# ChicyChen/LOCO-Edit

Hardware: AMD Instinct MI355X
Metric: edit-directions/sec (top-5 PMP-Jacobian SVD @256^2) + vT cos-sim vs ref (higher is better)
Workload: dtype bf16x3 (split-bf16 MFMA operands, fp32 accumulate + fp32 storage); 1 GPU; CelebA-HQ DDPM 256x256 top-5 local basis (l_eye-sized mask, L=2400), t=0.6T, 12 power iterations, one GPU; multi_gpu_form=single, probes_total=5, probes_per_gpu=5, kept=5, n_iter=12, mask_L=2400, weights=synthetic seed 0, streams=2

## Files before the change

loco-edit_amd/csrc/engine.hip:

```cpp
#include <hip/hip_runtime.h>

#include <algorithm>
#include <array>
#include <cmath>
#include <cstdio>
#include <cstdlib>
#include <cstring>
#include <map>
#include <memory>
#include <thread>
#include <atomic>
#include <string>
#include <vector>

#include "../../include/loco_hip.h"
#ifdef LOCO_DIAG
#include "../../include/loco_hip_diag.h"
#endif
#include "kernels.h"
#include "program.h"
#ifdef LOCO_DIAG
#include "conv_plan_text.h"
#endif

// ... 464 lines not shown
        switch (op.kind) {
            case OP_CONV_IN: case OP_CONV: case OP_DOWN: case OP_UP: case OP_OUT: convf(ow.conv, to.H, to.W); break;
            case OP_RES:
                convf(ow.c1, to.H, to.W); convf(ow.c2, to.H, to.W);
                if (op.has_nin) convf(ow.nin, to.H, to.W);
                break;
            case OP_XFMR: {
                for (const ConvP* p : {&ow.pj_in, &ow.qkvc, &ow.to_out1, &ow.xqc, &ow.to_out2, &ow.ff1, &ow.ff2, &ow.pj_out}) convf(*p, to.H, to.W);
                double T = (double)to.H * to.W;
                fl += 2.0 * 2.0 * T * T * to.C + 2.0 * 2.0 * T * c->cfg.context_len * to.C;
                break;
            }
            case OP_ATTN: {
                convf(ow.qkvc, to.H, to.W); convf(ow.proj, to.H, to.W);
                double T = (double)to.H * to.W;
                fl += 2.0 * 2.0 * T * T * to.C;
                if (op.has_x) {
                    convf(ow.xqc, to.H, to.W); convf(ow.xproj, to.H, to.W);
                    fl += 2.0 * 2.0 * T * c->cfg.context_len * to.C;
                }
                break;
            }
        }
    }
    W.flops = fl;
    for (auto& kv : c->params) { std::vector<float>().swap(kv.second.data); }
    return bind_weights(c);
}

struct Pass {
    loco_ctx* c;
    hipStream_t st;
    int B;
    float* arena;
    float* stats;
    float* T(int id) const { return arena + c->tens[id].off; }
    long bs() const { return c->prog->per_sample; }
};

static void drop_graphs(loco_ctx* c) {
    for (auto& kv : c->fwd_graphs) {
        if (kv.second.exec) (void)hipGraphExecDestroy(kv.second.exec);
        if (kv.second.graph) (void)hipGraphDestroy(kv.second.graph);
    }
    c->fwd_graphs.clear();
}
inline unsigned char* gemm_ws_get(loco_ctx* c, size_t need, hipStream_t st) {
    const int l = c->lane;
    if (c->gemm_ws_bytes[l] >= need) return c->gemm_ws[l];
    hipStreamCaptureStatus cs = hipStreamCaptureStatusNone;
    if (hipStreamIsCapturing(st, &cs) != hipSuccess || cs != hipStreamCaptureStatusNone) return nullptr;
    if (c->gemm_ws[l]) {
        (void)hipDeviceSynchronize();
        drop_graphs(c);
        (void)hipFree(c->gemm_ws[l]);
        c->bytes -= c->gemm_ws_bytes[l];
        c->gemm_ws[l] = nullptr; c->gemm_ws_bytes[l] = 0;
    }
    void* p = nullptr;
    if (hipMalloc(&p, need) != hipSuccess) { (void)hipGetLastError(); return nullptr; }
    c->gemm_ws[l] = static_cast<unsigned char*>(p); c->gemm_ws_bytes[l] = need; c->bytes += need;
    return c->gemm_ws[l];
}
inline void attn_note(loco_ctx* c, const char* kernel, const GemmArgs* g = nullptr) {
#ifdef LOCO_DIAG
    if (!c->attn_log) return;
    char line[192];
    if (g) snprintf(line, sizeof(line), "kernel=%s M=%d N=%d K=%d batch=%d heads=%d kcat=%d\n", kernel, g->M, g->N, g->K, g->batch,
                    g->batch2 > 0 ? g->batch2 : 1, g->A2 ? 1 : 0);
    else snprintf(line, sizeof(line), "kernel=%s\n", kernel);
    *c->attn_log += line;
#else
    (void)c; (void)kernel; (void)g;
#endif
}
inline bool attn_gemm_rec(const loco_ctx* c, const GemmArgs& g) { return c->prec >= 1 && c->gemm_lowp && gemm_rec_eligible(g); }
inline void attn_gemm_f32(loco_ctx* c, const GemmArgs& g, hipStream_t st) { attn_note(c, "gemm_f32", &g); launch_gemm(g, st); }
inline void attn_gemm(loco_ctx* c, const GemmArgs& g, hipStream_t st) {
    if (attn_gemm_rec(c, g)) {
        if (unsigned char* ws = gemm_ws_get(c, gemm_rec_ws_bytes(g), st)) { attn_note(c, "gemm_rec", &g); launch_gemm_rec(g, ws, st); return; }
    }
    if (c->prec >= 1 && c->gemm_lowp && gemm_prefers_bf16x3(g)) { attn_note(c, "gemm_bf16x3", &g); launch_gemm_bf16x3(g, st); }
    else attn_gemm_f32(c, g, st);
}
inline void attn_softmax_rows(loco_ctx* c, float* S, long rows, int T, hipStream_t st, int B, long bs) {
    attn_note(c, "softmax_rows"); launch_softmax_rows(S, rows, T, st, B, bs);
}
inline void attn_softmax_jac(loco_ctx* c, float* dS, const float* P, long rows, int T, float scale, hipStream_t st, int B, long bs) {
    attn_note(c, "softmax_jac"); launch_softmax_jac(dS, P, rows, T, rows, scale, st, B, bs);
}

void conv_defaults(ConvArgs& a) {
    std::memset(&a, 0, sizeof(a));
    a.stride = 1; a.pad = 1; a.nsplit = 1; a.mode = CM_NONE; a.res_scale = 1.f;
}

struct NS { float *sc, *sh, *mr, *tst, *tc; };
NS nstats(const loco_ctx* c, float* base, const NormP& n) {
    NS s;
    s.sc = base + n.soff; s.sh = s.sc + n.C; s.mr = s.sh + n.C; s.tst = s.mr + 2 * c->cfg.gn_groups;
    s.tc = s.tst + 2 * c->cfg.gn_groups;
    return s;
}

struct StatReq {
    int kind = ST_NONE;
    NormP* n = nullptr;
    float* stats = nullptr;
    const float* prim = nullptr;
    const float* ss_scale = nullptr; const float* ss_shift = nullptr;
    float* keep = nullptr; size_t keep_floats = 0; int* keep_ntile = nullptr;
};

void stats_standalone(loco_ctx* c, const StatReq& rq, const float* x, long xbs, int B, int HW, int s0, hipStream_t st) {
    const NormP& n = *rq.n;
    const long SB = c->prog->stats_per_sample;
    const int G = c->cfg.gn_groups;
    if (rq.kind == ST_FWD) {
        NS s = nstats(c, rq.stats + (long)s0 * SB, n);
        launch_gn_stats(x, xbs, B, n.C, HW, G, eps_of(c, n), n.gamma, n.beta, s.mr, s.sc, s.sh, SB, c->red, st, rq.ss_scale,
                        rq.ss_shift);
    } else {
        NS sp = nstats(c, c->statsP, n);
        NS stt = nstats(c, rq.stats + (long)s0 * SB, n);
        launch_gn_tstats(x, xbs, rq.prim, 0, B, n.C, HW, G, sp.sc, sp.sh, sp.mr, 0, 0, rq.kind == ST_TAN ? 0 : 1, stt.tst,
                         stt.tc, SB, c->red, st, c->cfg.act);
    }
}

bool run_conv(loco_ctx* c, const ConvArgs& a0, int taps, hipStream_t st, const StatReq* rq = nullptr,
              const ConvArgs* second = nullptr) {
    const size_t span = (size_t)c->cfg.max_batch * c->prog->per_sample;
    auto padded = [&](const float* p) { return (p >= c->arenaP && p < c->arenaP + span) || (p >= c->arenaT && p < c->arenaT + span); };
    ConvArgs a = a0, sc;
    a.act = c->cfg.act;
    if (a.mode == CM_GN_SILU && c->cfg.act == ACT_GELU) a.mode = CM_GN_GELU;
    a.in_padded = padded(a.in);
    if (second) { sc = *second; sc.in_padded = padded(sc.in); }
    ConvEnv e;
    e.prec = c->prec; e.chip_share = c->chip_share; e.lanes = c->lanes_active; e.lane_s0 = c->lane_s0;
    e.partial = c->partial; e.partial_floats = c->partial_floats; e.stpart = c->stpart; e.stpart_floats = c->stpart_floats;
    e.fuse_stats = c->fuse_stats; e.fuse_lin = c->fuse_lin; e.deep1 = c->deep1; e.max_batch = c->cfg.max_batch;
    StatAsk q;
    if (rq) {
        q.kind = rq->kind; q.norm = rq->n != nullptr; q.prim = rq->prim; q.keep = rq->keep; q.keep_floats = rq->keep_floats;
        if (rq->n && rq->n->sx_off >= 0 && c->sxcache) q.sx = c->sxcache + rq->n->sx_off;
    }
    const ConvPlan p = plan_conv(e, a, taps, rq ? &q : nullptr, second ? &sc : nullptr);
    if (p.sc_first) run_conv(c, *second, 1, st);
#ifdef LOCO_DIAG
    if (c->plan_log) conv_plan_text(p, taps, c->prec, *c->plan_log);
#endif
    if (rq && rq->kind != ST_NONE && rq->n) rq->n->ready = true;
    if (rq && rq->keep_ntile) *rq->keep_ntile = p.keep_ntile;
    const int HWo = a.Hout * a.Wout, Gn = c->cfg.gn_groups;
    const long SBs = c->prog->stats_per_sample;
    auto timed = [&](const char* name, double flops, const ConvArgs& y, auto&& launch) {
        loco_ctx::ProfRec r;
        if (c->prof_on) {
            r.name = name; r.flops = flops;
            r.cin = y.Cin; r.cout = y.Cout; r.h = y.Hout; r.b = y.B; r.ns = y.nsplit; r.mode = y.mode; r.taps = taps;
            r.e0 = c->next_event(); r.e1 = c->next_event();
            (void)hipEventRecord(r.e0, st);
        }
        launch();
        if (c->prof_on) { (void)hipEventRecord(r.e1, st); c->prof.push_back(r); }
// ... 223 lines not shown
                     float beta, const float* V2 = nullptr, long vb2 = 0, const float* S2 = nullptr, long sb2 = 0) {
    const int n = text ? s.Lt : s.T, col0 = text ? 0 : s.Lt;
    GemmArgs g; std::memset(&g, 0, sizeof(g));
    g.A = V; g.sam = n; g.sak = 1; g.sab = vb; g.sah = text ? s.KS : s.HS;
    g.Bm = S + col0; g.sbk = 1; g.sbn = s.Tk; g.sbb = sb; g.sbh = s.SS;
    g.C = O; g.scm = s.T; g.scn = 1; g.scb = ob; g.sch = oh;
    g.M = s.CH; g.N = s.T; g.K = n; g.batch = s.B; g.batch2 = s.NH; g.alpha = 1.f; g.beta = beta;
    g.A2 = V2; g.sab2 = vb2; g.Bm2 = S2 ? S2 + col0 : nullptr; g.sbb2 = sb2;
    return g;
}
GemmArgs attn_keys(const Attn& s, const float* X, long xb, long xh, const float* S, long sb, float* G, long gb) {
    GemmArgs g; std::memset(&g, 0, sizeof(g));
    g.A = X; g.sam = s.T; g.sak = 1; g.sab = xb; g.sah = xh;
    g.Bm = S + s.Lt; g.sbk = s.Tk; g.sbn = 1; g.sbb = sb; g.sbh = s.SS;
    g.C = G; g.scm = s.T; g.scn = 1; g.scb = gb; g.sch = s.HS;
    g.M = s.CH; g.N = s.T; g.K = s.T; g.batch = s.B; g.batch2 = s.NH; g.alpha = 1.f; g.beta = 0.f;
    return g;
}
AttnFlashArgs attn_flash_args(const Attn& s) {
    AttnFlashArgs fa; std::memset(&fa, 0, sizeof(fa));
    fa.ws = s.ws; fa.ws_bytes = s.ws_bytes;
    fa.T = s.T; fa.NH = s.NH; fa.B = s.B; fa.CH = s.CH; fa.scale = s.scale;
    fa.q = s.q; fa.k = s.k; fa.v = s.v; fa.hs = s.HS;
    fa.P = s.P; fa.o = s.o;
    if (s.Lt) { fa.Lt = s.Lt; fa.kt = s.kt; fa.vt = s.vt; }
    return fa;
}
inline void attn_note_flash(loco_ctx* c, const AttnFlashArgs& fa, bool tan) {
#ifdef LOCO_DIAG
    if (!c->attn_log) return;
    const bool dma = attn_flash_dma_route(fa.ws, fa.ws_bytes, attn_flash_ws_bytes(fa), attn_flash_dma_enabled());
    if (dma) attn_note(c, "attn_split");
    if (tan) attn_note(c, dma ? "flash_dma_tan" : "flash_tan");
    else { attn_note(c, dma ? "flash_dma_cotq" : "flash_cotq"); attn_note(c, dma ? "flash_dma_cotk" : "flash_cotk"); }
#else
    (void)c; (void)fa; (void)tan;
#endif
}
void attn_forward(const Attn& s) {
    loco_ctx* c = s.c;
    float *q = s.tq, *k = s.tk, *v = s.tv, *S = s.tS, *o = s.to;
    if (s.Lt) attn_gemm_f32(c, attn_scores(s, TEXT, q, s.bq, s.HS, s.kt, 0, S, s.bS, s.scale, 0.f, true), s.st);
    attn_gemm(c, attn_scores(s, IMAGE, q, s.bq, s.HS, k, s.bq, S, s.bS, s.scale, 0.f), s.st);
    attn_softmax_rows(c, S, (long)s.NH * s.T, s.Tk, s.st, s.B, s.bS);
    attn_gemm(c, attn_values(s, IMAGE, v, s.bq, S, s.bS, o, s.bo, s.OS, 0.f), s.st);
    if (s.Lt) attn_gemm_f32(c, attn_values(s, TEXT, s.vt, 0, S, s.bS, o, s.bo, s.OS, 1.f), s.st);
}
void attn_tangent(const Attn& s) {
    loco_ctx* c = s.c;
    const float *q = s.q, *k = s.k, *v = s.v, *SP = s.P;
    float *dq = s.tq, *dk = s.tk, *dv = s.tv, *ST = s.tS, *oT = s.to;
    if (s.flash()) {
        AttnFlashArgs fa = attn_flash_args(s);
        fa.dq = dq; fa.dk = dk; fa.dv = dv; fa.bs_d = s.bq; fa.out = oT; fa.bs_out = s.bo;
        attn_note_flash(c, fa, true);
        launch_attn_flash_tangent(fa, s.st);
        return;
    }
    const GemmArgs dS2 = attn_scores(s, IMAGE, dq, s.bq, s.HS, k, 0, ST, s.bS, 1.f, 0.f, false, q, 0, dk, s.bq);
    const bool kcat = s.pair && (s.T <= 256 || attn_gemm_rec(c, dS2));
    if (s.Lt) attn_gemm_f32(c, attn_scores(s, TEXT, dq, s.bq, s.HS, s.kt, 0, ST, s.bS, 1.f, 0.f), s.st);
    if (kcat) attn_gemm(c, dS2, s.st);
    else {
        attn_gemm(c, attn_scores(s, IMAGE, dq, s.bq, s.HS, k, 0, ST, s.bS, 1.f, 0.f), s.st);
        attn_gemm(c, attn_scores(s, IMAGE, q, 0, s.HS, dk, s.bq, ST, s.bS, 1.f, 1.f), s.st);
    }
    attn_softmax_jac(c, ST, SP, (long)s.NH * s.T, s.Tk, s.scale, s.st, s.B, s.bS);
    if (kcat) attn_gemm(c, attn_values(s, IMAGE, dv, s.bq, SP, 0, oT, s.bo, s.OS, 0.f, v, 0, ST, s.bS), s.st);
    else {
        attn_gemm(c, attn_values(s, IMAGE, dv, s.bq, SP, 0, oT, s.bo, s.OS, 0.f), s.st);
        attn_gemm(c, attn_values(s, IMAGE, v, 0, ST, s.bS, oT, s.bo, s.OS, 1.f), s.st);
    }
    if (s.Lt) attn_gemm_f32(c, attn_values(s, TEXT, s.vt, 0, ST, s.bS, oT, s.bo, s.OS, 1.f), s.st);
}
void attn_cotangent(const Attn& s) {
    loco_ctx* c = s.c;
    const float *q = s.q, *k = s.k, *v = s.v, *SP = s.P;
    float *gq = s.tq, *gk = s.tk, *gv = s.tv, *SG = s.tS, *oG = s.to;
    if (s.flash()) {
        AttnFlashArgs fa = attn_flash_args(s);
        fa.go = oG; fa.bs_go = s.bo; fa.gq = gq; fa.gk = gk; fa.gv = gv; fa.bs_g = s.bq; fa.delta = s.delta;
        attn_note_flash(c, fa, false);
        launch_attn_flash_cotangent(fa, s.st);
        return;
    }
    attn_gemm(c, attn_keys(s, oG, s.bo, s.OS, SP, 0, gv, s.bq), s.st);
    if (s.Lt) attn_gemm_f32(c, attn_scores(s, TEXT, oG, s.bo, s.OS, s.vt, 0, SG, s.bS, 1.f, 0.f), s.st);
    attn_gemm(c, attn_scores(s, IMAGE, oG, s.bo, s.OS, v, 0, SG, s.bS, 1.f, 0.f), s.st);
    attn_softmax_jac(c, SG, SP, (long)s.NH * s.T, s.Tk, s.scale, s.st, s.B, s.bS);
    attn_gemm(c, attn_values(s, IMAGE, k, 0, SG, s.bS, gq, s.bq, s.HS, 0.f), s.st);
    if (s.Lt) attn_gemm_f32(c, attn_values(s, TEXT, s.kt, 0, SG, s.bS, gq, s.bq, s.HS, 1.f), s.st);
    attn_gemm(c, attn_keys(s, q, 0, s.HS, SG, s.bS, gk, s.bq), s.st);
}

void lin1x1(loco_ctx* c, const ConvP& w, bool dgrad, const float* in, long in_bs, int Cin, float* out, long out_bs, int Cout,
            int H, int W, int B, const float* res, long res_bs, bool with_bias, hipStream_t st, const StatReq* rq = nullptr) {
    ConvArgs a; conv_defaults(a);
    a.in = in; a.in_bs = in_bs; a.Cin = Cin; a.Hin = H; a.Win = W;
    setw(a, w, dgrad); a.pad = 0;
    if (with_bias) a.bias = w.bias;
    a.res = res; a.res_bs = res_bs;
    a.out = out; a.out_bs = out_bs; a.Cout = Cout; a.Hout = H; a.Wout = W; a.B = B;
    run_conv(c, a, 1, st, rq);
}

int forward_pass(loco_ctx* c, const float* x, float t, int B, float* arena, float* stats, hipStream_t st,
                 const float* t_ptr = nullptr) {
    const loco_unet_cfg& cfg = c->cfg;
    Pass p{c, st, B, arena, stats};
    const long SB = c->prog->stats_per_sample;
    clear_ready(c);
    auto next_fwd = [&](int tid) { return req_fwd_of(c, tid, stats); };
    if (cfg.arch < 2) {
        launch_temb(t, cfg.ch, cfg.ch * 4, c->wts->freq, c->wts->td0w, c->wts->td0b, c->wts->td1w, c->wts->td1b, c->tact, st, cfg.arch == 1,
                    c->has_cond ? c->cond_add : nullptr, t_ptr, cfg.act, c->has_tcond ? c->cond_in : nullptr);
        launch_temb_proj(c->tact, cfg.ch * 4, c->wts->tp_w, c->wts->tp_b, (int)c->wts->tproj_total, c->tproj, st);
    }
    for (auto& op : c->ops) {
        const Tens& to = c->tens[op.out];
        const int HW = to.H * to.W;
        switch (op.kind) {
            case OP_CONV_IN: {
                ConvArgs a; conv_defaults(a);
                a.in = x; a.in_bs = c->prog->n_in; a.Cin = cfg.in_channels; a.Hin = cfg.resolution; a.Win = cfg.resolution;
                setw(a, op.conv, false); a.bias = op.conv.bias;
                a.out = p.T(op.out); a.out_bs = p.bs(); a.Cout = to.C; a.Hout = to.H; a.Wout = to.W; a.B = B;
                if (op.ksize == 1) a.pad = 0;
                const StatReq rq = next_fwd(op.out);
                run_conv(c, a, op.ksize == 1 ? 1 : 9, st, &rq);
                break;
            }
            case OP_CONV: {
                const Tens& ti = c->tens[op.in];
                ConvArgs a; conv_defaults(a);
                a.in = p.T(op.in); a.in_bs = p.bs(); a.Cin = ti.C; a.Hin = ti.H; a.Win = ti.W;
                setw(a, op.conv, false); a.bias = op.conv.bias;
                a.out = p.T(op.out); a.out_bs = p.bs(); a.Cout = to.C; a.Hout = to.H; a.Wout = to.W; a.B = B;
                if (op.ksize == 1) a.pad = 0;
                const StatReq rq = next_fwd(op.out);
                run_conv(c, a, op.ksize == 1 ? 1 : 9, st, &rq);
                break;
            }
            case OP_RES: {
                const Tens& ti = c->tens[op.in];
                const int HWi = ti.H * ti.W;
                if (!op.n1.ready && !cat_fused_stats(c, op.n1, op.in, stats, B, st)) gn_forward_stats(p, op.n1, p.T(op.in), p.bs(), HWi);
                op.n1.ready = false;
                NS s1 = nstats(c, stats, op.n1);
                ConvArgs a; conv_defaults(a);
                a.Cin = ti.C;
                setw(a, op.c1, false); a.bias = op.c1.bias;
                if (!op.scale_shift && op.has_temb) { a.bias2 = c->tproj + op.tproj_off; a.bias2_bs = 0; }
                if (op.updown == 1) {
                    launch_gn_apply(4, nullptr, 0, p.T(op.in), p.bs(), nullptr, 0, p.T(op.a1), p.bs(), 0, B, ti.C, HWi,
                                    cfg.gn_groups, s1.sc, s1.sh, s1.mr, SB, SB, nullptr, 0, st, cfg.act);
                    launch_pool2x2_sum(p.T(op.a1), p.bs(), p.T(op.ap), p.bs(), 0, B, ti.C, to.H, to.W, st, 0.25f);
                    launch_pool2x2_sum(p.T(op.in), p.bs(), p.T(op.xu), p.bs(), 0, B, ti.C, to.H, to.W, st, 0.25f);
                    a.in = p.T(op.ap); a.in_bs = p.bs(); a.Hin = to.H; a.Win = to.W;
                } else {
                    a.in = p.T(op.in); a.in_bs = p.bs(); a.Hin = ti.H; a.Win = ti.W;
                    a.mode = CM_GN_SILU; a.sc = s1.sc; a.sh = s1.sh; a.scsh_bs = SB;
                    if (op.updown == 2) {
                        a.upsample = 1;
                        launch_upsample2x(p.T(op.in), p.bs(), p.T(op.xu), p.bs(), 0, 1.0f, B, ti.C, ti.H, ti.W, st);
                    }
                }
// ... 1900 lines not shown
```

loco-edit_amd/csrc/gemm.hip:

```cpp
#include "kernels.h"
#include <cstdlib>

namespace loco {

typedef float f32x16 __attribute__((ext_vector_type(16)));

constexpr int GBM = 64, GBN = 64, GBK = 64;

template <int NSEG, int EPI = GEMM_ACT_NONE>
__global__ __launch_bounds__(256) void gemm_f32_kernel(GemmArgs g) {
    __shared__ float As[GBK][GBM + 1];
    __shared__ float Bs[GBK][GBN + 1];
    const int tid = threadIdx.x, lane = tid & 63, wave = tid >> 6;
    const int l31 = lane & 31, khalf = lane >> 5;
    const int wm = wave >> 1, wn = wave & 1;
    const int m0 = blockIdx.y * GBM, n0 = blockIdx.x * GBN;
    const int nb2 = g.batch2 > 0 ? g.batch2 : 1;
    const int bz = blockIdx.z / nb2, hz = blockIdx.z % nb2;
    const float* A = g.A + (long)bz * g.sab + (long)hz * g.sah;
    const float* B = g.Bm + (long)bz * g.sbb + (long)hz * g.sbh;
    f32x16 acc;
#pragma unroll
    for (int r = 0; r < 16; ++r) acc[r] = 0.f;

    constexpr int NE = GBM * GBK / 256;
    int am[NE], ak[NE], bn[NE], bk[NE];
#pragma unroll
    for (int i = 0; i < NE; ++i) {
        int e = tid + i * 256;
        if (g.sak == 1) { am[i] = e / GBK; ak[i] = e % GBK; } else { ak[i] = e / GBM; am[i] = e % GBM; }
        if (g.sbn == 1) { bk[i] = e / GBN; bn[i] = e % GBN; } else { bn[i] = e / GBK; bk[i] = e % GBK; }
    }
    float ra[NE], rb[NE];
    auto fetch = [&](int k0) {
#pragma unroll
        for (int i = 0; i < NE; ++i) {
            bool va = (m0 + am[i] < g.M) && (k0 + ak[i] < g.K);
            bool vb = (n0 + bn[i] < g.N) && (k0 + bk[i] < g.K);
            long oa = va ? (long)(m0 + am[i]) * g.sam + (long)(k0 + ak[i]) * g.sak : 0;
            long ob = vb ? (long)(k0 + bk[i]) * g.sbk + (long)(n0 + bn[i]) * g.sbn : 0;
            float xa = A[oa], xb = B[ob];
            ra[i] = va ? xa : 0.f;
            rb[i] = vb ? xb : 0.f;
        }
    };
#pragma unroll
    for (int seg = 0; seg < NSEG; ++seg) {
        if (seg) {
            A = g.A2 + (long)bz * g.sab2 + (long)hz * g.sah;
            B = g.Bm2 + (long)bz * g.sbb2 + (long)hz * g.sbh;
        }
        fetch(0);
        for (int k0 = 0; k0 < g.K; k0 += GBK) {
            __syncthreads();
#pragma unroll
            for (int i = 0; i < NE; ++i) { As[ak[i]][am[i]] = ra[i]; Bs[bk[i]][bn[i]] = rb[i]; }
            __syncthreads();
            if (k0 + GBK < g.K) fetch(k0 + GBK);
#pragma unroll
            for (int kk = 0; kk < GBK / 2; ++kk) {
                float a = As[2 * kk + khalf][wm * 32 + l31];
                float b = Bs[2 * kk + khalf][wn * 32 + l31];
                acc = __builtin_amdgcn_mfma_f32_32x32x2f32(a, b, acc, 0, 0, 0);
            }
        }
    }
    const int n = n0 + wn * 32 + l31;
    if (n < g.N) {
#pragma unroll
        for (int r = 0; r < 16; ++r) {
            int m = m0 + wm * 32 + (r & 3) + 8 * (r >> 2) + 4 * khalf;
            if (m >= g.M) continue;
            long off = (long)m * g.scm + (long)n * g.scn;
            float v = g.alpha * acc[r];
            float* c = g.C + (long)bz * g.scb + (long)hz * g.sch + off;
            if (g.beta != 0.f) v += g.beta * (*c);
            if (g.bias) v += g.bias[m];
                if (g.colbias) v += g.colbias[n];
            if (g.R) v += g.R[(long)bz * g.srb + (long)hz * g.sch + off];
            if (EPI == GEMM_ACT_QUICK_GELU) v = v * (1.0f / (1.0f + expf(-1.702f * v)));
            else if (EPI == GEMM_ACT_GELU) v = 0.5f * v * (1.0f + erff(v * 0.70710678118654752f));
            *c = v;
        }
    }
}

constexpr int SBM = 32, SBN = 32, SBK = 64;
template <int NSEG>
__global__ __launch_bounds__(256) void gemm_f32_small_kernel(GemmArgs g) {
    __shared__ float As[SBK][SBM + 1];
    __shared__ float Bs[SBK][SBN + 1];
    __shared__ float Red[3][16][64];
    const int tid = threadIdx.x, lane = tid & 63, wave = tid >> 6;
    const int l31 = lane & 31, khalf = lane >> 5;
    const int m0 = blockIdx.y * SBM, n0 = blockIdx.x * SBN;
    const int nb2 = g.batch2 > 0 ? g.batch2 : 1;
    const int bz = blockIdx.z / nb2, hz = blockIdx.z % nb2;
    const float* A = g.A + (long)bz * g.sab + (long)hz * g.sah;
    const float* B = g.Bm + (long)bz * g.sbb + (long)hz * g.sbh;
    f32x16 acc;
#pragma unroll
    for (int r = 0; r < 16; ++r) acc[r] = 0.f;
    constexpr int NE = SBM * SBK / 256;
    int am[NE], ak[NE], bn[NE], bk[NE];
#pragma unroll
    for (int i = 0; i < NE; ++i) {
        int e = tid + i * 256;
        if (g.sak == 1) { am[i] = e / SBK; ak[i] = e % SBK; } else { ak[i] = e / SBM; am[i] = e % SBM; }
        if (g.sbn == 1) { bk[i] = e / SBN; bn[i] = e % SBN; } else { bn[i] = e / SBK; bk[i] = e % SBK; }
    }
    float ra[NE], rb[NE];
    auto fetch = [&](int k0) {
#pragma unroll
        for (int i = 0; i < NE; ++i) {
            bool va = (m0 + am[i] < g.M) && (k0 + ak[i] < g.K);
            bool vb = (n0 + bn[i] < g.N) && (k0 + bk[i] < g.K);
            long oa = va ? (long)(m0 + am[i]) * g.sam + (long)(k0 + ak[i]) * g.sak : 0;
            long ob = vb ? (long)(k0 + bk[i]) * g.sbk + (long)(n0 + bn[i]) * g.sbn : 0;
            float xa = A[oa], xb = B[ob];
            ra[i] = va ? xa : 0.f;
            rb[i] = vb ? xb : 0.f;
        }
    };
#pragma unroll
    for (int seg = 0; seg < NSEG; ++seg) {
        if (seg) {
            A = g.A2 + (long)bz * g.sab2 + (long)hz * g.sah;
            B = g.Bm2 + (long)bz * g.sbb2 + (long)hz * g.sbh;
        }
        fetch(0);
        for (int k0 = 0; k0 < g.K; k0 += SBK) {
            __syncthreads();
#pragma unroll
            for (int i = 0; i < NE; ++i) { As[ak[i]][am[i]] = ra[i]; Bs[bk[i]][bn[i]] = rb[i]; }
            __syncthreads();
            if (k0 + SBK < g.K) fetch(k0 + SBK);
#pragma unroll
            for (int kk = 0; kk < SBK / 8; ++kk) {
                float a = As[2 * (wave * (SBK / 8) + kk) + khalf][l31];
                float b = Bs[2 * (wave * (SBK / 8) + kk) + khalf][l31];
                acc = __builtin_amdgcn_mfma_f32_32x32x2f32(a, b, acc, 0, 0, 0);
            }
        }
    }
    if (wave > 0) {
#pragma unroll
        for (int r = 0; r < 16; ++r) Red[wave - 1][r][lane] = acc[r];
    }
    __syncthreads();
    if (wave > 0) return;
#pragma unroll
    for (int w = 0; w < 3; ++w)
#pragma unroll
        for (int r = 0; r < 16; ++r) acc[r] += Red[w][r][lane];
    const int n = n0 + l31;
    if (n < g.N) {
#pragma unroll
        for (int r = 0; r < 16; ++r) {
            int m = m0 + (r & 3) + 8 * (r >> 2) + 4 * khalf;
            if (m >= g.M) continue;
            long off = (long)m * g.scm + (long)n * g.scn;
            float v = g.alpha * acc[r];
            float* c = g.C + (long)bz * g.scb + (long)hz * g.sch + off;
            if (g.beta != 0.f) v += g.beta * (*c);
            if (g.bias) v += g.bias[m];
            if (g.colbias) v += g.colbias[n];
            if (g.R) v += g.R[(long)bz * g.srb + (long)hz * g.sch + off];
            *c = v;
        }
    }
}

typedef __bf16 bf16x8_g __attribute__((ext_vector_type(8)));

__device__ __forceinline__ void split_pair(float a, float b, unsigned& hi, unsigned& lo) {
    typedef float f32x2_ __attribute__((ext_vector_type(2)));
    typedef __bf16 bf16x2_ __attribute__((ext_vector_type(2)));
    hi = __builtin_bit_cast(unsigned, __builtin_convertvector((f32x2_){a, b}, bf16x2_));
    const float ha = __builtin_bit_cast(float, hi << 16), hb = __builtin_bit_cast(float, hi & 0xffff0000u);
    float da = a - ha;
    asm volatile("" : "+v"(da));
    const float db = b - hb;
    lo = __builtin_bit_cast(unsigned, __builtin_convertvector((f32x2_){da, db}, bf16x2_));
}
__device__ __forceinline__ void split_piece(const float* v, uint4& hi, uint4& lo) {
    split_pair(v[0], v[1], hi.x, lo.x);
    split_pair(v[2], v[3], hi.y, lo.y);
    split_pair(v[4], v[5], hi.z, lo.z);
    split_pair(v[6], v[7], hi.w, lo.w);
}
__device__ __forceinline__ int grec(int row, int piece) { return row * 64 + ((piece ^ ((row >> 2) & 3)) << 4); }

template <int BM, int BN, int NSEG>
__global__ __launch_bounds__(256) void gemm_bf16x3_kernel(GemmArgs g) {
    constexpr int BK = 32, KS = BK / 16;
    constexpr int TM = BM / 64, TN = BN / 64;
    constexpr int NA = BM * 4 / 256, NB = BN * 4 / 256;
    __shared__ __attribute__((aligned(16))) unsigned char As[KS * BM * 64];
    __shared__ __attribute__((aligned(16))) unsigned char Bs[KS * BN * 64];
    const int tid = threadIdx.x, lane = tid & 63, wave = tid >> 6;
    const int l31 = lane & 31, khalf = lane >> 5;
    const int wm = wave >> 1, wn = wave & 1;
    const int m0 = blockIdx.y * BM, n0 = blockIdx.x * BN;
    const int nb2 = g.batch2 > 0 ? g.batch2 : 1;
    const int bz = blockIdx.z / nb2, hz = blockIdx.z % nb2;
    const float* A = g.A + (long)bz * g.sab + (long)hz * g.sah;
    const float* B = g.Bm + (long)bz * g.sbb + (long)hz * g.sbh;
    f32x16 acc[TM][TN];
#pragma unroll
    for (int i = 0; i < TM; ++i)
#pragma unroll
        for (int j = 0; j < TN; ++j)
#pragma unroll
            for (int r = 0; r < 16; ++r) acc[i][j][r] = 0.f;

    float ra[NA][8], rb[NB][8];
    auto fetch = [&](int k0) {
#pragma unroll
        for (int it = 0; it < NA; ++it) {
            const int e = tid + it * 256, m = e % BM, kq = e / BM;
            const bool vm = m0 + m < g.M;
#pragma unroll
            for (int j = 0; j < 8; ++j) {
                const int k = k0 + kq * 8 + j;
                const bool v = vm && k < g.K;
                const float x = A[v ? (long)(m0 + m) * g.sam + (long)k * g.sak : 0];
                ra[it][j] = v ? x : 0.f;
            }
        }
#pragma unroll
        for (int it = 0; it < NB; ++it) {
            const int e = tid + it * 256, n = e % BN, kq = e / BN;
            const bool vn = n0 + n < g.N;
#pragma unroll
            for (int j = 0; j < 8; ++j) {
                const int k = k0 + kq * 8 + j;
                const bool v = vn && k < g.K;
                const float x = B[v ? (long)k * g.sbk + (long)(n0 + n) * g.sbn : 0];
                rb[it][j] = v ? x : 0.f;
            }
        }
    };
#pragma unroll
    for (int seg = 0; seg < NSEG; ++seg) {
    if (seg) {
        A = g.A2 + (long)bz * g.sab2 + (long)hz * g.sah;
        B = g.Bm2 + (long)bz * g.sbb2 + (long)hz * g.sbh;
    }
    fetch(0);
    for (int k0 = 0; k0 < g.K; k0 += BK) {
        __syncthreads();
#pragma unroll
// ... 3 lines not shown
            split_piece(ra[it], hi, lo);
            unsigned char* rec = As + (kq >> 1) * BM * 64;
            *reinterpret_cast<uint4*>(rec + grec(m, kq & 1)) = hi;
            *reinterpret_cast<uint4*>(rec + grec(m, 2 + (kq & 1))) = lo;
        }
#pragma unroll
        for (int it = 0; it < NB; ++it) {
            const int e = tid + it * 256, n = e % BN, kq = e / BN;
            uint4 hi, lo;
            split_piece(rb[it], hi, lo);
            unsigned char* rec = Bs + (kq >> 1) * BN * 64;
            *reinterpret_cast<uint4*>(rec + grec(n, kq & 1)) = hi;
            *reinterpret_cast<uint4*>(rec + grec(n, 2 + (kq & 1))) = lo;
        }
        __syncthreads();
        if (k0 + BK < g.K) fetch(k0 + BK);
#pragma unroll
        for (int ks = 0; ks < KS; ++ks) {
            bf16x8_g ah[TM], al[TM], bh[TN], bl[TN];
#pragma unroll
            for (int i = 0; i < TM; ++i) {
                const int m = (wm * TM + i) * 32 + l31;
                ah[i] = *reinterpret_cast<const bf16x8_g*>(As + ks * BM * 64 + grec(m, khalf));
                al[i] = *reinterpret_cast<const bf16x8_g*>(As + ks * BM * 64 + grec(m, 2 + khalf));
            }
#pragma unroll
            for (int j = 0; j < TN; ++j) {
                const int n = (wn * TN + j) * 32 + l31;
                bh[j] = *reinterpret_cast<const bf16x8_g*>(Bs + ks * BN * 64 + grec(n, khalf));
                bl[j] = *reinterpret_cast<const bf16x8_g*>(Bs + ks * BN * 64 + grec(n, 2 + khalf));
            }
#pragma unroll
            for (int i = 0; i < TM; ++i)
#pragma unroll
                for (int j = 0; j < TN; ++j) {
                    acc[i][j] = __builtin_amdgcn_mfma_f32_32x32x16_bf16(al[i], bh[j], acc[i][j], 0, 0, 0);
                    acc[i][j] = __builtin_amdgcn_mfma_f32_32x32x16_bf16(ah[i], bl[j], acc[i][j], 0, 0, 0);
                    acc[i][j] = __builtin_amdgcn_mfma_f32_32x32x16_bf16(ah[i], bh[j], acc[i][j], 0, 0, 0);
                }
        }
    }
    }
#pragma unroll
    for (int i = 0; i < TM; ++i)
#pragma unroll
        for (int j = 0; j < TN; ++j) {
            const int n = n0 + (wn * TN + j) * 32 + l31;
            if (n >= g.N) continue;
#pragma unroll
            for (int r = 0; r < 16; ++r) {
                const int m = m0 + (wm * TM + i) * 32 + (r & 3) + 8 * (r >> 2) + 4 * khalf;
                if (m >= g.M) continue;
                const long off = (long)m * g.scm + (long)n * g.scn;
                float v = g.alpha * acc[i][j][r];
                float* c = g.C + (long)bz * g.scb + (long)hz * g.sch + off;
                if (g.beta != 0.f) v += g.beta * (*c);
                if (g.bias) v += g.bias[m];
                if (g.colbias) v += g.colbias[n];
                if (g.R) v += g.R[(long)bz * g.srb + (long)hz * g.sch + off];
                *c = v;
            }
        }
}

bool gemm_prefers_bf16x3(const GemmArgs& g) {
    const double macs = (double)g.M * g.N * g.K * (g.A2 ? 2 : 1) * g.batch * (g.batch2 > 0 ? g.batch2 : 1);
    return g.K >= 256 && macs >= 4e9;
}

void launch_gemm_bf16x3(const GemmArgs& g, hipStream_t st) {
    const int nb = g.batch * (g.batch2 > 0 ? g.batch2 : 1);
    const long big = (long)((g.N + 127) / 128) * ((g.M + 127) / 128) * nb;
    if (big >= 512 && g.M >= 128 && g.N >= 128) {
        dim3 grid((g.N + 127) / 128, (g.M + 127) / 128, nb);
        if (g.A2) hipLaunchKernelGGL((gemm_bf16x3_kernel<128, 128, 2>), grid, dim3(256), 0, st, g);
        else hipLaunchKernelGGL((gemm_bf16x3_kernel<128, 128, 1>), grid, dim3(256), 0, st, g);
    } else {
        dim3 grid((g.N + 63) / 64, (g.M + 63) / 64, nb);
        if (g.A2) hipLaunchKernelGGL((gemm_bf16x3_kernel<64, 64, 2>), grid, dim3(256), 0, st, g);
        else hipLaunchKernelGGL((gemm_bf16x3_kernel<64, 64, 1>), grid, dim3(256), 0, st, g);
    }
}

void launch_gemm(const GemmArgs& g, hipStream_t st) {
    const int nz = g.batch * (g.batch2 > 0 ? g.batch2 : 1);
    static int small_on = -1;
    if (small_on < 0) { const char* e = getenv("LOCO_GEMM_SMALL"); small_on = e ? (atoi(e) != 0) : 1; }
    const long wg64 = (long)((g.N + GBN - 1) / GBN) * ((g.M + GBM - 1) / GBM) * nz;
    static int small_wg = -1;
    if (small_wg < 0) { const char* e = getenv("LOCO_GEMM_SMALL_WG"); small_wg = e ? atoi(e) : 320; }
    if (small_on && wg64 < small_wg && g.K >= 128) {
        dim3 sg((g.N + SBN - 1) / SBN, (g.M + SBM - 1) / SBM, nz);
        if (g.A2) hipLaunchKernelGGL(gemm_f32_small_kernel<2>, sg, dim3(256), 0, st, g);
        else hipLaunchKernelGGL(gemm_f32_small_kernel<1>, sg, dim3(256), 0, st, g);
        return;
    }
    dim3 grid((g.N + GBN - 1) / GBN, (g.M + GBM - 1) / GBM, g.batch * (g.batch2 > 0 ? g.batch2 : 1));
    if (g.A2) hipLaunchKernelGGL(gemm_f32_kernel<2>, grid, dim3(256), 0, st, g);
    else hipLaunchKernelGGL(gemm_f32_kernel<1>, grid, dim3(256), 0, st, g);
}

void launch_gemm_fixed(const GemmArgs& g, int act, hipStream_t st) {
    dim3 grid((g.N + GBN - 1) / GBN, (g.M + GBM - 1) / GBM, g.batch * (g.batch2 > 0 ? g.batch2 : 1));
    if (g.A2) hipLaunchKernelGGL(gemm_f32_kernel<2>, grid, dim3(256), 0, st, g);
    else if (act == GEMM_ACT_QUICK_GELU) hipLaunchKernelGGL((gemm_f32_kernel<1, GEMM_ACT_QUICK_GELU>), grid, dim3(256), 0, st, g);
    else if (act == GEMM_ACT_GELU) hipLaunchKernelGGL((gemm_f32_kernel<1, GEMM_ACT_GELU>), grid, dim3(256), 0, st, g);
    else hipLaunchKernelGGL(gemm_f32_kernel<1>, grid, dim3(256), 0, st, g);
}

}
```

loco-edit_amd/csrc/kernels.h:

```cpp
#pragma once
#include <hip/hip_runtime.h>
#include <stdint.h>

namespace loco {

struct DeviceOnce { bool seen[64] = {}; };
inline bool first_on_device(DeviceOnce& f) {
    int d = 0;
    (void)hipGetDevice(&d);
    d &= 63;
    if (f.seen[d]) return false;
    f.seen[d] = true;
    return true;
}


enum ConvMode : int {
    CM_NONE = 0,
    CM_GN_SILU = 1,
    CM_GN = 2,
    CM_TAN_SILU = 3,
    CM_COT_SILU = 4,
    CM_GN_GELU = 5,
};
// ... 52 lines not shown
    const void* wpb; const void* wph;
    int poly;
    int pool2; float* pool_tmp; long pool_tmp_bs;
    const void* wqb; const void* wqh;
};

enum PolyKind : int { POLY_UP = 0, POLY_ZINS_PAD2 = 1, POLY_ZINS_PAD1 = 2 };
inline int polyphase_vcout(int C, int a, int b, int co) { return ((a * (C / 64) + co / 64) * 2 + b) * 64 + (co % 64); }
void polyphase_fold(int kind, int nin, int nout, const float* w, long so, long si, long st, float* out);
void polyphase_fold_in(int nin, int nout, const float* w, long so, long si, long st, float* out, int noutP);

void launch_conv(const ConvArgs& a, int taps, hipStream_t st);
void launch_conv_bf16x3(const ConvArgs& a, int taps, hipStream_t st);
void launch_conv_f16(const ConvArgs& a, int taps, hipStream_t st);
void launch_conv_splitk_reduce(const ConvArgs& a, hipStream_t st);

struct ConvEnv {
    int prec = 1;
    int chip_share = 1;
    int lanes = 1, lane_s0 = 0;
    float* partial = nullptr; size_t partial_floats = 0;
    float* stpart = nullptr; size_t stpart_floats = 0;
    bool fuse_stats = true, fuse_lin = true, deep1 = true;
    int max_batch = 1;
};

struct StatAsk {
    int kind = ST_NONE;
    bool norm = false;
    const float2* sx = nullptr;
    const float* prim = nullptr;
    float* keep = nullptr; size_t keep_floats = 0;
};

enum StatRoute : int {
    SR_NONE = 0,
    SR_EPI = 1,
    SR_SPLITK = 2,
    SR_ALONE = 3,
    SR_KEEP = 4,
};

struct ConvLaunch {
    ConvArgs args;
    int s0 = 0;
    int stats = SR_NONE;
    int ntile = 0;
};

struct ConvPlan {
    bool sc_first = false;
    int nl = 1;
    ConvLaunch l[2];
    bool stats_all = false;
    int keep_ntile = 0;
    bool pool_after = false; float* pool_out = nullptr; long pool_out_bs = 0; int pool_acc = 0;
    bool cot = false;
};

ConvPlan plan_conv(const ConvEnv& env, const ConvArgs& a, int taps, const StatAsk* ask, const ConvArgs* shortcut);
void conv_plan_family(ConvArgs& a, int prec);
void conv_plan_tile_pair(ConvArgs& a, int prec, int tile_override);

int conv_bf16_tile_couts(const ConvArgs& a);
const char* conv_variant_name(const ConvArgs& a, int taps, int prec);

void launch_fill_random(float* p, long count, unsigned seed, float scale, hipStream_t st);
void launch_gn_cache(const float* x, int C, int HW, int cpg, const float* sc, const float* sh, const float* mr,
                     float2* sx, hipStream_t st, int act = 0);

struct GemmArgs {
    const float* A; long sam, sak, sab;
    const float* Bm; long sbk, sbn, sbb;
    float* C; long scm, scn, scb;
    const float* bias;
    const float* colbias;
    const float* R; long srb;
    int M, N, K, batch;
    float alpha, beta;
    int batch2; long sah, sbh, sch;
    const float* A2; long sab2; const float* Bm2; long sbb2;
};
void launch_gemm(const GemmArgs& g, hipStream_t st);
enum GemmAct : int { GEMM_ACT_NONE = 0, GEMM_ACT_QUICK_GELU = 1, GEMM_ACT_GELU = 2 };
void launch_gemm_fixed(const GemmArgs& g, int act, hipStream_t st);
void launch_gemm_bf16x3(const GemmArgs& g, hipStream_t st);
bool gemm_prefers_bf16x3(const GemmArgs& g);
bool gemm_rec_eligible(const GemmArgs& g);
size_t gemm_rec_ws_bytes(const GemmArgs& g);
void launch_gemm_rec(const GemmArgs& g, unsigned char* ws, hipStream_t st);

struct AttnFlashArgs {
    int T, NH, B, CH; float scale;
    const float *q, *k, *v; long hs;
    const float* P;
    const float* o;
    const float *dq, *dk, *dv; long bs_d;
    float* out; long bs_out;
    const float* go; long bs_go;
    float *gq, *gk, *gv; long bs_g;
    float* delta;
    int Lt; const float *kt, *vt;
    unsigned char* ws; size_t ws_bytes;
};
size_t attn_flash_ws_bytes(const AttnFlashArgs& a);
inline bool attn_flash_dma_route(const unsigned char* ws, size_t ws_bytes, size_t need, bool dma_on) {
    return ws != nullptr && dma_on && need <= ws_bytes;
}
bool attn_flash_dma_enabled();
bool attn_flash_supported(int T, int CH);
bool attn_flash_text_supported(int T, int CH, int Lt);
void launch_attn_flash_tangent(const AttnFlashArgs& a, hipStream_t st);
void launch_attn_flash_cotangent(const AttnFlashArgs& a, hipStream_t st);

void launch_ln_fwd(const float* x, long xbs, int B, int C, int T, const float* gamma, const float* beta, float eps, float* y,
                   long ybs, float* stats, long sbs, hipStream_t st);
void launch_ln_tan(const float* dx, long dbs, const float* xprim, const float* sprim, int B, int C, int T, const float* gamma,
                   float* dy, long ybs, hipStream_t st);
void launch_ln_cot(const float* gy, long gbs, const float* xprim, const float* sprim, int B, int C, int T, const float* gamma,
                   const float* base, long base_bs, float* gx, long xbs, hipStream_t st);
struct XAttnArgs {
    int T, NH, B, CH, L, Lp, fwd;
    float alpha;
    const float* X; long x_bs;
    const float* K1; const float* K2;
    float* P; long p_bs;
    float* O; long o_bs;
};
bool xattn_fused_supported(int T, int CH, int L, int Lp);
void launch_xattn_fused(const XAttnArgs& a, hipStream_t st);
void launch_geglu(int kind, const float* in, long in_bs, const float* fprim, int B, long n4, float* out, long out_bs,
                  hipStream_t st);

void launch_gn_stats(const float* x, long bs, int B, int C, int HW, int G, float eps,
                     const float* gamma, const float* beta,
                     float* mr, float* sc, float* sh, long stats_bs, double* scratch, hipStream_t st,
                     const float* ss_scale = nullptr, const float* ss_shift = nullptr);
void launch_gn_fused_finalize_cat(const float* partA, int C1, int ntA, const float* partB, int ntB, int B, int C, int HW, int G,
                                  float eps, const float* gamma, const float* beta, float* mr, float* sc, float* sh,
                                  long stats_bs, hipStream_t st);
void launch_gn_fused_finalize(const float* part, int ntile, int B, int C, int HW, int G, float eps, const float* gamma,
                              const float* beta, float* mr, float* sc, float* sh, long stats_bs, const float* ss_scale,
                              const float* ss_shift, hipStream_t st);
void launch_gn_lin_fused_finalize(int kind, const float* partA, int C1, int ntA, const float* partB, int ntB, int B, int C, int HW,
                                  int G, const float* mr, float* tst, float* tc, long tst_bs, hipStream_t st);
void launch_conv_splitk_reduce_stats(const ConvArgs& a, int kind, int G, float eps, const float* gamma, const float* beta,
                                     float* mr, float* sc, float* sh, long stats_bs, const float* ss_scale,
                                     const float* ss_shift, const float* prim, const float* sc_prim, const float* sh_prim,
                                     const float* mr_prim, float* tst, float* tc, long tst_bs, double* scratch,
                                     hipStream_t st);
void launch_gn_tstats(const float* d, long d_bs, const float* x, long x_bs, int B, int C, int HW, int G,
                      const float* sc, const float* sh, const float* mr, long pbs_c, long pbs_g,
                      int kind, float* tst, float* tc, long tst_bs, double* scratch, hipStream_t st, int act = 0);
void launch_gn_apply(int kind, const float* d, long d_bs, const float* x, long x_bs,
                     const float* base, long base_bs, float* out, long out_bs, int accumulate,
                     int B, int C, int HW, int G, const float* sc, const float* sh, const float* mr,
                     long pbs_c, long pbs_g, const float* tst, long tst_bs, hipStream_t st, int act = 0,
                     float base_scale = 1.0f);

void launch_ctx_groupnorm(const float* tok, int L, int D, int G, float eps, const float* gamma, const float* beta,
                          float* out, hipStream_t st);

void launch_softmax_rows(float* S, long rows, int T, hipStream_t st, int B = 1, long bs = 0);
void launch_softmax_jac(float* dS, const float* P, long rows, int T, long p_rows, float scale, hipStream_t st,
                        int B = 1, long bs = 0);

// ... 79 lines not shown
```

Measured before the change: 20.50 edit-directions/s.

## Add register-prefetched small fp32 GEMM and grouped two-GEMM launch for attention cotangent

Adds a double-buffered small fp32 GEMM kernel that prefetches the next K-tile into registers while MFMAs run on the current LDS stage. It is specialised on whether each operand is K-major, and used when shapes divide the tile and pointers are 16-byte aligned. Independent GEMM pairs in the non-flash attention cotangent (gv with dS scores, gq with gk) are also grouped into a single launch that splits the z-grid between the two problems. The aim is to hide global-load latency and to fill more CUs with small attention GEMMs. The cost is more template instantiations and idle blocks when the paired GEMMs differ in size.

Measured after the change: 20.71 edit-directions/s (median of 6 runs). 1.0% higher.

```diff
diff --git a/loco-edit_amd/csrc/engine.hip b/loco-edit_amd/csrc/engine.hip
--- a/loco-edit_amd/csrc/engine.hip
+++ b/loco-edit_amd/csrc/engine.hip
@@ -570,6 +570,12 @@
     }
     if (c->prec >= 1 && c->gemm_lowp && gemm_prefers_bf16x3(g)) { attn_note(c, "gemm_bf16x3", &g); launch_gemm_bf16x3(g, st); }
     else attn_gemm_f32(c, g, st);
+}
+inline void attn_gemm_pair(loco_ctx* c, const GemmArgs& g0, const GemmArgs& g1, hipStream_t st) {
+    auto f32 = [&](const GemmArgs& g) { return !attn_gemm_rec(c, g) && !(c->prec >= 1 && c->gemm_lowp && gemm_prefers_bf16x3(g)); };
+    if (!f32(g0) || !f32(g1)) { attn_gemm(c, g0, st); attn_gemm(c, g1, st); return; }
+    attn_note(c, "gemm_f32", &g0); attn_note(c, "gemm_f32", &g1);
+    launch_gemm_pair(g0, g1, st);
 }
 inline void attn_softmax_rows(loco_ctx* c, float* S, long rows, int T, hipStream_t st, int B, long bs) {
     attn_note(c, "softmax_rows"); launch_softmax_rows(S, rows, T, st, B, bs);
@@ -959,6 +965,14 @@
         fa.go = oG; fa.bs_go = s.bo; fa.gq = gq; fa.gk = gk; fa.gv = gv; fa.bs_g = s.bq; fa.delta = s.delta;
         attn_note_flash(c, fa, false);
         launch_attn_flash_cotangent(fa, s.st);
+        return;
+    }
+    if (!s.Lt) {
+        attn_gemm_pair(c, attn_keys(s, oG, s.bo, s.OS, SP, 0, gv, s.bq),
+                       attn_scores(s, IMAGE, oG, s.bo, s.OS, v, 0, SG, s.bS, 1.f, 0.f), s.st);
+        attn_softmax_jac(c, SG, SP, (long)s.NH * s.T, s.Tk, s.scale, s.st, s.B, s.bS);
+        attn_gemm_pair(c, attn_values(s, IMAGE, k, 0, SG, s.bS, gq, s.bq, s.HS, 0.f),
+                       attn_keys(s, q, 0, s.HS, SG, s.bS, gk, s.bq), s.st);
         return;
     }
     attn_gemm(c, attn_keys(s, oG, s.bo, s.OS, SP, 0, gv, s.bq), s.st);
diff --git a/loco-edit_amd/csrc/gemm.hip b/loco-edit_amd/csrc/gemm.hip
--- a/loco-edit_amd/csrc/gemm.hip
+++ b/loco-edit_amd/csrc/gemm.hip
@@ -1,9 +1,11 @@
 #include "kernels.h"
+#include <cstdint>
 #include <cstdlib>
 
 namespace loco {
 
 typedef float f32x16 __attribute__((ext_vector_type(16)));
+typedef float f32x4 __attribute__((ext_vector_type(4)));
 
 constexpr int GBM = 64, GBN = 64, GBK = 64;
 
@@ -168,6 +170,125 @@
             if (g.R) v += g.R[(long)bz * g.srb + (long)hz * g.sch + off];
             *c = v;
         }
+    }
+}
+
+constexpr int PKM_LD = SBM + 4, PMM_LD = SBK + 1;
+constexpr int PSTAGE = SBK * PKM_LD;
+static_assert(PSTAGE >= SBM * PMM_LD && 4 * PSTAGE >= 3 * 16 * 64, "stage buffers hold either layout and the reduction buffer");
+
+template <bool KM>
+__device__ __forceinline__ void pipe_thread_map(int tid, int r0, long srow, long sk, long& off, long& d, long& adv) {
+    if (KM) { off = (long)(tid >> 3) * sk + r0 + (tid & 7) * 4; d = 32 * sk; adv = SBK * sk; }
+    else { off = (long)(r0 + (tid >> 4)) * srow + (tid & 15) * 4; d = 16 * srow; adv = SBK; }
+}
+template <bool KM>
+__device__ __forceinline__ void pipe_stage(float* st, int tid, const f32x4 (&r)[2]) {
+#pragma unroll
+    for (int i = 0; i < 2; ++i) {
+        if (KM) *reinterpret_cast<f32x4*>(st + ((tid >> 3) + 32 * i) * PKM_LD + (tid & 7) * 4) = r[i];
+        else {
+            float* p = st + ((tid >> 4) + 16 * i) * PMM_LD + (tid & 15) * 4;
+            p[0] = r[i][0]; p[1] = r[i][1]; p[2] = r[i][2]; p[3] = r[i][3];
+        }
+    }
+}
+
+template <int NSEG, bool AKM, bool BKM>
+__device__ __forceinline__ void gemm_f32_small_pipe_body(const GemmArgs& g, int z, float* smem) {
+    const int tid = threadIdx.x, lane = tid & 63, wave = tid >> 6;
+    const int l31 = lane & 31, khalf = lane >> 5;
+    const int m0 = blockIdx.y * SBM, n0 = blockIdx.x * SBN;
+    const int nb2 = g.batch2 > 0 ? g.batch2 : 1;
+    const int bz = z / nb2, hz = z % nb2;
+    float* sA = smem;
+    float* sB = smem + 2 * PSTAGE;
+    long offA, dA, advA, offB, dB, advB;
+    pipe_thread_map<AKM>(tid, m0, g.sam, g.sak, offA, dA, advA);
+    pipe_thread_map<BKM>(tid, n0, g.sbn, g.sbk, offB, dB, advB);
+    const float* pA = g.A + (long)bz * g.sab + (long)hz * g.sah + offA;
+    const float* pB = g.Bm + (long)bz * g.sbb + (long)hz * g.sbh + offB;
+    const int nk = g.K / SBK, total = NSEG * nk;
+    int left = nk;
+    auto load = [&](f32x4 (&ra)[2], f32x4 (&rb)[2]) {
+        ra[0] = *reinterpret_cast<const f32x4*>(pA); ra[1] = *reinterpret_cast<const f32x4*>(pA + dA);
+        rb[0] = *reinterpret_cast<const f32x4*>(pB); rb[1] = *reinterpret_cast<const f32x4*>(pB + dB);
+        pA += advA; pB += advB;
+        if (NSEG == 2 && --left == 0) {
+            pA = g.A2 + (long)bz * g.sab2 + (long)hz * g.sah + offA;
+            pB = g.Bm2 + (long)bz * g.sbb2 + (long)hz * g.sbh + offB;
+        }
+    };
+    f32x16 acc;
+#pragma unroll
+    for (int r = 0; r < 16; ++r) acc[r] = 0.f;
+    const int kq0 = wave * (SBK / 4) + khalf;
+    const int fa0 = AKM ? kq0 * PKM_LD + l31 : l31 * PMM_LD + kq0, fas = AKM ? 2 * PKM_LD : 2;
+    const int fb0 = BKM ? kq0 * PKM_LD + l31 : l31 * PMM_LD + kq0, fbs = BKM ? 2 * PKM_LD : 2;
+    auto mma = [&](int buf) {
+        const float* as = sA + buf * PSTAGE + fa0;
+        const float* bs = sB + buf * PSTAGE + fb0;
+#pragma unroll
+        for (int kk = 0; kk < SBK / 8; ++kk) acc = __builtin_amdgcn_mfma_f32_32x32x2f32(as[kk * fas], bs[kk * fbs], acc, 0, 0, 0);
+    };
+    f32x4 ra[2][2], rb[2][2];
+    load(ra[0], rb[0]);
+    load(ra[1], rb[1]);
+    pipe_stage<AKM>(sA, tid, ra[0]); pipe_stage<BKM>(sB, tid, rb[0]);
+    __syncthreads();
+    for (int t = 0; t < total; t += 2) {
+        if (t + 2 < total) load(ra[0], rb[0]);
+        mma(0);
+        if (t + 1 < total) { pipe_stage<AKM>(sA + PSTAGE, tid, ra[1]); pipe_stage<BKM>(sB + PSTAGE, tid, rb[1]); }
+        __syncthreads();
+        if (t + 1 >= total) break;
+        if (t + 3 < total) load(ra[1], rb[1]);
+        mma(1);
+        if (t + 2 < total) { pipe_stage<AKM>(sA, tid, ra[0]); pipe_stage<BKM>(sB, tid, rb[0]); }
+        __syncthreads();
+    }
+    float (*Red)[16][64] = reinterpret_cast<float (*)[16][64]>(smem);
+    if (wave > 0) {
+#pragma unroll
+        for (int r = 0; r < 16; ++r) Red[wave - 1][r][lane] = acc[r];
+    }
+    __syncthreads();
+    if (wave > 0) return;
+#pragma unroll
+    for (int w = 0; w < 3; ++w)
+#pragma unroll
+        for (int r = 0; r < 16; ++r) acc[r] += Red[w][r][lane];
+    const int n = n0 + l31;
+    float* cb = g.C + (long)bz * g.scb + (long)hz * g.sch;
+    const float* rbp = g.R ? g.R + (long)bz * g.srb + (long)hz * g.sch : nullptr;
+#pragma unroll
+    for (int r = 0; r < 16; ++r) {
+        const int m = m0 + (r & 3) + 8 * (r >> 2) + 4 * khalf;
+        const long off = (long)m * g.scm + (long)n * g.scn;
+        float v = g.alpha * acc[r];
+        float* c = cb + off;
+        if (g.beta != 0.f) v += g.beta * (*c);
+        if (g.bias) v += g.bias[m];
+        if (g.colbias) v += g.colbias[n];
+        if (rbp) v += rbp[off];
+        *c = v;
+    }
+}
+
+template <int NSEG, bool AKM, bool BKM>
+__global__ __launch_bounds__(256) void gemm_f32_small_pipe_kernel(GemmArgs g) {
+    __shared__ __attribute__((aligned(16))) float smem[4 * PSTAGE];
+    gemm_f32_small_pipe_body<NSEG, AKM, BKM>(g, blockIdx.z, smem);
+}
+template <bool AKM0, bool BKM0, bool AKM1, bool BKM1>
+__global__ __launch_bounds__(256) void gemm_f32_small_pipe2_kernel(GemmArgs g0, GemmArgs g1, int nz0) {
+    __shared__ __attribute__((aligned(16))) float smem[4 * PSTAGE];
+    if ((int)blockIdx.z < nz0) {
+        if ((int)blockIdx.x * SBN >= g0.N || (int)blockIdx.y * SBM >= g0.M) return;
+        gemm_f32_small_pipe_body<1, AKM0, BKM0>(g0, blockIdx.z, smem);
+    } else {
+        if ((int)blockIdx.x * SBN >= g1.N || (int)blockIdx.y * SBM >= g1.M) return;
+        gemm_f32_small_pipe_body<1, AKM1, BKM1>(g1, blockIdx.z - nz0, smem);
     }
 }
 
@@ -337,16 +458,70 @@
     }
 }
 
-void launch_gemm(const GemmArgs& g, hipStream_t st) {
+static bool gemm_small_taken(const GemmArgs& g) {
     const int nz = g.batch * (g.batch2 > 0 ? g.batch2 : 1);
     static int small_on = -1;
     if (small_on < 0) { const char* e = getenv("LOCO_GEMM_SMALL"); small_on = e ? (atoi(e) != 0) : 1; }
     const long wg64 = (long)((g.N + GBN - 1) / GBN) * ((g.M + GBM - 1) / GBM) * nz;
     static int small_wg = -1;
     if (small_wg < 0) { const char* e = getenv("LOCO_GEMM_SMALL_WG"); small_wg = e ? atoi(e) : 320; }
-    if (small_on && wg64 < small_wg && g.K >= 128) {
+    return small_on && wg64 < small_wg && g.K >= 128;
+}
+static bool gemm_small_pipe_eligible(const GemmArgs& g) {
+    static int pipe_on = -1;
+    if (pipe_on < 0) { const char* e = getenv("LOCO_GEMM_SMALL_PIPE"); pipe_on = e ? (atoi(e) != 0) : 1; }
+    if (!pipe_on || g.M % SBM || g.N % SBN || g.K % SBK || g.K < 2 * SBK) return false;
+    auto al = [](const float* p) { return (reinterpret_cast<uintptr_t>(p) & 15) == 0; };
+    auto op = [&](long s1, long s2, long sb, long sh, const float* p, const float* p2, long sb2) {
+        const long so = s1 == 1 ? s2 : s1;
+        if ((s1 != 1 && s2 != 1) || so % 4 || sb % 4 || sh % 4 || !al(p)) return false;
+        return !g.A2 || (sb2 % 4 == 0 && al(p2));
+    };
+    return op(g.sam, g.sak, g.sab, g.sah, g.A, g.A2, g.sab2) && op(g.sbn, g.sbk, g.sbb, g.sbh, g.Bm, g.Bm2, g.sbb2);
+}
+template <int NSEG>
+static void launch_small_pipe(const GemmArgs& g, dim3 sg, hipStream_t st) {
+    const bool akm = g.sam == 1, bkm = g.sbn == 1;
+    if (akm && bkm) hipLaunchKernelGGL((gemm_f32_small_pipe_kernel<NSEG, true, true>), sg, dim3(256), 0, st, g);
+    else if (akm) hipLaunchKernelGGL((gemm_f32_small_pipe_kernel<NSEG, true, false>), sg, dim3(256), 0, st, g);
+    else if (bkm) hipLaunchKernelGGL((gemm_f32_small_pipe_kernel<NSEG, false, true>), sg, dim3(256), 0, st, g);
+    else hipLaunchKernelGGL((gemm_f32_small_pipe_kernel<NSEG, false, false>), sg, dim3(256), 0, st, g);
+}
+template <bool AKM0, bool BKM0>
+static void launch_small_pipe2(const GemmArgs& g0, const GemmArgs& g1, dim3 sg, int nz0, hipStream_t st) {
+    const bool akm = g1.sam == 1, bkm = g1.sbn == 1;
+    if (akm && bkm) hipLaunchKernelGGL((gemm_f32_small_pipe2_kernel<AKM0, BKM0, true, true>), sg, dim3(256), 0, st, g0, g1, nz0);
+    else if (akm) hipLaunchKernelGGL((gemm_f32_small_pipe2_kernel<AKM0, BKM0, true, false>), sg, dim3(256), 0, st, g0, g1, nz0);
+    else if (bkm) hipLaunchKernelGGL((gemm_f32_small_pipe2_kernel<AKM0, BKM0, false, true>), sg, dim3(256), 0, st, g0, g1, nz0);
+    else hipLaunchKernelGGL((gemm_f32_small_pipe2_kernel<AKM0, BKM0, false, false>), sg, dim3(256), 0, st, g0, g1, nz0);
+}
+
+void launch_gemm_pair(const GemmArgs& g0, const GemmArgs& g1, hipStream_t st) {
+    static int group_on = -1;
+    if (group_on < 0) { const char* e = getenv("LOCO_GEMM_GROUP"); group_on = e ? (atoi(e) != 0) : 1; }
+    if (!group_on || g0.A2 || g1.A2 || !gemm_small_taken(g0) || !gemm_small_taken(g1) || !gemm_small_pipe_eligible(g0) ||
+        !gemm_small_pipe_eligible(g1)) {
+        launch_gemm(g0, st);
+        launch_gemm(g1, st);
+        return;
+    }
+    const int nz0 = g0.batch * (g0.batch2 > 0 ? g0.batch2 : 1), nz1 = g1.batch * (g1.batch2 > 0 ? g1.batch2 : 1);
+    dim3 sg((g0.N > g1.N ? g0.N : g1.N) / SBN, (g0.M > g1.M ? g0.M : g1.M) / SBM, nz0 + nz1);
+    const bool akm = g0.sam == 1, bkm = g0.sbn == 1;
+    if (akm && bkm) launch_small_pipe2<true, true>(g0, g1, sg, nz0, st);
+    else if (akm) launch_small_pipe2<true, false>(g0, g1, sg, nz0, st);
+    else if (bkm) launch_small_pipe2<false, true>(g0, g1, sg, nz0, st);
+    else launch_small_pipe2<false, false>(g0, g1, sg, nz0, st);
+}
+
+void launch_gemm(const GemmArgs& g, hipStream_t st) {
+    const int nz = g.batch * (g.batch2 > 0 ? g.batch2 : 1);
+    if (gemm_small_taken(g)) {
         dim3 sg((g.N + SBN - 1) / SBN, (g.M + SBM - 1) / SBM, nz);
-        if (g.A2) hipLaunchKernelGGL(gemm_f32_small_kernel<2>, sg, dim3(256), 0, st, g);
+        if (gemm_small_pipe_eligible(g)) {
+            if (g.A2) launch_small_pipe<2>(g, sg, st);
+            else launch_small_pipe<1>(g, sg, st);
+        } else if (g.A2) hipLaunchKernelGGL(gemm_f32_small_kernel<2>, sg, dim3(256), 0, st, g);
         else hipLaunchKernelGGL(gemm_f32_small_kernel<1>, sg, dim3(256), 0, st, g);
         return;
     }
diff --git a/loco-edit_amd/csrc/kernels.h b/loco-edit_amd/csrc/kernels.h
--- a/loco-edit_amd/csrc/kernels.h
+++ b/loco-edit_amd/csrc/kernels.h
@@ -158,6 +158,7 @@
     const float* A2; long sab2; const float* Bm2; long sbb2;
 };
 void launch_gemm(const GemmArgs& g, hipStream_t st);
+void launch_gemm_pair(const GemmArgs& g0, const GemmArgs& g1, hipStream_t st);
 enum GemmAct : int { GEMM_ACT_NONE = 0, GEMM_ACT_QUICK_GELU = 1, GEMM_ACT_GELU = 2 };
 void launch_gemm_fixed(const GemmArgs& g, int act, hipStream_t st);
 void launch_gemm_bf16x3(const GemmArgs& g, hipStream_t st);
```
